# ctSkennerton/crass

Measured on AMD Instinct MI355X. Metric: reads/sec through DR search+recruit, 150bp synthetic, 1/2/4/8 MI355X, higher is better.
Workload: dtype u8; 1 GPU; 100000000 synthetic 150 bp reads, 50 seeded DRs, 1 % CRISPR reads (BASELINE.json configs[2]); pass1 + merge + pass2; total_reads=100000000, reads_per_gpu=100000000, read_len=150, n_dr=50, parallelism=read-shards x1, launcher=single context, pass1_found=563794, pass2_found=436000, patterns=13320, ac_states=0, filter_survivors=1705594, fast_filter=1, lds_automaton=2, merge_fallbacks=0

## Files before the change

### crass_amd/build.py

```python
import os
import shutil
import subprocess
import sys

HERE = os.path.dirname(os.path.abspath(__file__))
CSRC = os.path.join(HERE, "csrc")
LIB = os.path.join(HERE, "libcrass_hip.so")
SOURCES = ["kernels.hip", "pass2.hip", "sinks.hip", "dmerge.hip", "consensus.hip", "pack.hip", "fastx_scan.hip", "fastx_names.hip", "inflate.hip", "gunzip.hip", "engine.cpp", "engine_ingest.cpp", "merge.cpp", "ingest.cpp", "fastx_scan.cpp", "bgzf.cpp", "gunzip.cpp", "consensus.cpp", "group.cpp", "graph.cpp", "sdma.cpp", "pgzip.cpp"]
HEADERS = ["engine_internal.h", "engine_ctx.h", "dev_common.h", "comp_table.h", "devmem.h", "pack_text.h", "lane_find.h", "pack_launch.h", "fastx_scan.h", "fastx_launch.h", "fastx_names_launch.h", "inflate_core.h", "inflate_launch.h", "gunzip_core.h", "gunzip_launch.h", "consensus_internal.h", "merge.h", os.path.join("..", "..", "include", "crass_hip.h")]


def _hipcc():
    for cand in (os.environ.get("HIPCC"), shutil.which("hipcc"), "/opt/rocm/bin/hipcc"):
        if cand and os.path.exists(cand):
            return cand
    raise RuntimeError("hipcc not found: the MI355X engine cannot be built")


OBJ = os.path.join(CSRC, "_obj")
FLAGS = ["--offload-arch=gfx950", "-O3", "-std=c++17", "-ffp-contract=off", "-fPIC", "-Wall", "-Wno-unused-function"]
LIBS = ["-lz", "-lpthread", "-ldl"]


def _stale(target, deps):
    if not os.path.exists(target):
        return True
    t = os.path.getmtime(target)
    return any(os.path.getmtime(d) > t for d in deps)


def needs_build():
    return _stale(LIB, [os.path.join(CSRC, d) for d in SOURCES + HEADERS])


def build(force=False, verbose=False):
    if not force and not needs_build():
        return LIB
    os.makedirs(OBJ, exist_ok=True)
    hipcc = _hipcc()
    hdrs = [os.path.join(CSRC, h) for h in HEADERS]
    jobs = []
    objs = []
    for s in SOURCES:
        src, obj = os.path.join(CSRC, s), os.path.join(OBJ, s + ".o")
        objs.append(obj)
        if force or _stale(obj, [src] + hdrs):
            cmd = [hipcc] + FLAGS + ["-x", "hip", "-c", src, "-o", obj]
            if verbose:
                print(" ".join(cmd), file=sys.stderr)
            jobs.append((s, subprocess.Popen(cmd, stdout=subprocess.PIPE, stderr=subprocess.STDOUT, text=True)))
    failed = []
    for s, p in jobs:
        out, _ = p.communicate()
        if out.strip():
            print(out, file=sys.stderr, end="")
        if p.returncode:
            failed.append(s)
    if failed:
        raise RuntimeError("hipcc failed for: " + ", ".join(failed))
    tmp = LIB + ".tmp"
    cmd = [hipcc, "--offload-arch=gfx950", "-shared", "-fPIC", "-o", tmp] + objs + LIBS
    if verbose:
        print(" ".join(cmd), file=sys.stderr)
    subprocess.check_call(cmd)
    from . import vgpr_guard
    try:
        vgpr_guard.check(tmp)
    except Exception:
        os.replace(tmp, LIB + ".rejected")
        raise
    os.replace(tmp, LIB)
    return LIB


ADAPTER_DIR = os.path.join(CSRC, "adapter")
CLI = os.path.join(HERE, "crass-hip")
ADAPTER_LIB = os.path.join(HERE, "libcrass_adapter.so")


def build_adapter(force=False, verbose=False):
    build(force=force, verbose=verbose)
    srcs = [os.path.join(ADAPTER_DIR, "crass_adapter.cpp")]
    deps = srcs + [os.path.join(ADAPTER_DIR, "crass_adapter.h"), os.path.join(ADAPTER_DIR, "crass_hip_cli.cpp"), LIB]
    if not force and os.path.exists(CLI) and os.path.exists(ADAPTER_LIB) and \
            all(os.path.getmtime(d) <= min(os.path.getmtime(CLI), os.path.getmtime(ADAPTER_LIB)) for d in deps):
        return CLI
    cxx = shutil.which("g++") or "g++"
    common = [cxx, "-O2", "-std=c++17", "-Wall", "-fPIC", "-pthread"]
    rpath = ["-L" + HERE, "-lcrass_hip", "-Wl,-rpath," + HERE, "-Wl,-rpath,$ORIGIN"]
    for cmd in (common + ["-shared", "-o", ADAPTER_LIB] + srcs + rpath,
                common + ["-o", CLI, os.path.join(ADAPTER_DIR, "crass_hip_cli.cpp")] + srcs + rpath):
        if verbose:
            print(" ".join(cmd), file=sys.stderr)
        subprocess.check_call(cmd)
    return CLI


if __name__ == "__main__":
    print(build(force="--force" in sys.argv, verbose=True))
    print(build_adapter(force="--force" in sys.argv, verbose=True))
```

### crass_amd/csrc/engine.cpp

```cpp
#include "engine_ctx.h"

#include <cstdio>
#include <new>
#include <string>

void crass_hip_ctx::widen_p1() const
{
    P1Dense &D = dense;
    if (D.wide_ready) return;
    (void)wait_bulk();
    const uint64_t n = D.n;
    const uint32_t ss_cap = D.pack_ss_cap, stride = dr_stride;
    const uint8_t *hb = D.h_blob.p;
    const uint16_t *b_replen = (const uint16_t *)(hb + D.lay.replen), *b_ss = (const uint16_t *)(hb + D.lay.ss);
    const uint8_t *b_nss = hb + D.lay.nss, *b_ss8 = hb + D.lay.ss;
    D.w_replen.resize(n); D.w_nss.resize(n); D.w_ss_off.resize(n); D.w_ss.resize(n * (size_t)ss_cap);
    D.w_dr_len.resize(n); D.w_dr.resize(n * (size_t)stride);
    if (D.dr_fallback) (void)hipStreamSynchronize(copy_stream);
    else (void)wait_dx();
    const size_t per_task = 16384;
    host_parallel_for((size_t)((n + per_task - 1) / per_task), 16, [&](size_t t) {
        const uint64_t k0 = t * per_task, k1 = std::min<uint64_t>(n, k0 + per_task);
        for (uint64_t k = k0; k < k1; k++) { D.w_replen[k] = b_replen[k]; D.w_nss[k] = b_nss[k]; D.w_ss_off[k] = k * (uint64_t)ss_cap; }
        if (D.lay.ss_elem == 1) for (uint64_t i = k0 * ss_cap; i < k1 * (uint64_t)ss_cap; i++) D.w_ss[i] = b_ss8[i];
        else for (uint64_t i = k0 * ss_cap; i < k1 * (uint64_t)ss_cap; i++) D.w_ss[i] = b_ss[i];
        if (D.dr_fallback) {
            memcpy(D.w_dr.data() + k0 * (size_t)stride, D.h_dr_fb.p + k0 * (size_t)stride, (size_t)(k1 - k0) * stride);
            memcpy(D.w_dr_len.data() + k0, D.h_dr_len_fb.p + k0, (size_t)(k1 - k0) * 2);
        } else {
            for (uint64_t k = k0; k < k1; k++) {
                const uint32_t j = h_dmap.p[k];
                memcpy(D.w_dr.data() + k * (size_t)stride, h_dx_chars.p + j * (size_t)stride, stride);
                D.w_dr_len[k] = h_dx_len.p[j];
            }
        }
    });
    D.wide_ready = true;
}

static void quiesce_worker(crass_hip_ctx *c)
{
    if (c->dm.build_pending) {
        if (!c->worker.run_here_if_not_started()) c->worker.wait();
        c->dm.build_pending = false;
        (void)c->worker.take_failed();
        c->dm.br.valid = false;
        if (c->dm.br.hip) { c->last_hip = c->dm.br.hip; c->dm.br.hip = 0; }
    }
}

static bool getenv_once_copy_early()
{
    static const bool on = getenv("CRASS_COPY_EARLY") != nullptr;
    return on;
}


extern "C" {

int crass_hip_abi_version(void) { return CRASS_HIP_ABI_VERSION; }

int crassi_anchor_shape(uint32_t low_dr, uint32_t *key_bases, uint32_t *align_bases)
{
    uint32_t kb = 0, ash = 0;
    const bool ok = dm_anchor_shape(low_dr, kb, ash);
    if (key_bases) *key_bases = ok ? kb : 0u;
    if (align_bases) *align_bases = ok ? 1u << ash : 0u;
    return ok ? 1 : 0;
}

uint64_t crassi_dev_bytes_live(void) { return g_dev_bytes.load(std::memory_order_relaxed); }

void crass_default_params(crass_params *p)
{
    p->lowDRsize = 23; p->highDRsize = 47; p->lowSpacerSize = 26; p->highSpacerSize = 50;
    p->searchWindowLength = 8; p->minNumRepeats = 2; p->kmer_clust_size = 6;
}

const char *crass_hip_strerror(int s)
{
    switch (s) {
        case CRASS_OK: return "ok";
        case CRASS_ERR_INVALID_ARG: return "invalid argument";
        case CRASS_ERR_UNSUPPORTED: return "parameter outside the device path's implementation limits";
        case CRASS_ERR_NO_DEVICE: return "no usable HIP device";
        case CRASS_ERR_HIP: return "HIP runtime call failed";
        case CRASS_ERR_OOM: return "out of memory";
        case CRASS_ERR_STATE: return "call order violated";
        case CRASS_ERR_SEARCH_FATAL: return "Fatal error in search algorithm!";
        case CRASS_ERR_OVERFLOW: return "device pool overflow";
        case CRASS_ERR_IO: return "I/O error";
        case CRASS_ERR_RCCL: return "RCCL call failed (crass_hip_group_last_error())";
        default: return "unknown status";
    }
}

int crass_hip_last_hip_error(const crass_hip_ctx *ctx) { return ctx ? ctx->last_hip : 0; }
void *crass_hip_stream(const crass_hip_ctx *ctx) { return ctx ? (void *)ctx->stream : nullptr; }

int crass_hip_create(const crass_params *p, int device, crass_hip_ctx **out)
{
    if (!p || !out) return CRASS_ERR_INVALID_ARG;
    *out = nullptr;
    if (p->searchWindowLength < CRASS_HIP_MIN_WINDOW || p->searchWindowLength > CRASS_HIP_MAX_WINDOW) return CRASS_ERR_INVALID_ARG;
    if (p->lowDRsize < 8 || p->lowSpacerSize < 8) return CRASS_ERR_INVALID_ARG;
    if (p->lowDRsize >= p->highDRsize || p->lowSpacerSize >= p->highSpacerSize) return CRASS_ERR_INVALID_ARG;
    if (p->minNumRepeats < 2) return CRASS_ERR_INVALID_ARG;
    if (p->highDRsize > CRASS_HIP_MAX_DR) return CRASS_ERR_UNSUPPORTED;
    if (p->lowDRsize < 2 * p->searchWindowLength - 1) return CRASS_ERR_UNSUPPORTED;
    int ndev = 0;
    if (hipGetDeviceCount(&ndev) != hipSuccess || ndev <= 0 || device < 0 || device >= ndev) return CRASS_ERR_NO_DEVICE;
    crass_hip_ctx *c = new (std::nothrow) crass_hip_ctx();
    if (!c) return CRASS_ERR_OOM;
    c->prm = *p;
    c->device = device;
    c->dp.lowDR = p->lowDRsize; c->dp.highDR = p->highDRsize; c->dp.lowSp = p->lowSpacerSize; c->dp.highSp = p->highSpacerSize;
    c->dp.window = p->searchWindowLength; c->dp.minRepeats = p->minNumRepeats;
    uint32_t skips = p->lowDRsize - (2 * p->searchWindowLength - 1);
    if (skips < 1) skips = 1;
    c->dp.skips = skips;
    c->env.read();
    g_dev_cap.store(c->env.pool_cap_bytes, std::memory_order_relaxed);
    c->dp.debug_stop = c->env.surv_debug;
    c->dp.find_serial = c->env.lane_find_serial ? 1u : 0u;
    if (c->env.stage_timing >= 0) c->timing_level = c->env.stage_timing;
    if (c->env.no_lookback) c->lb_on = false;
    c->dr_stride = (p->highDRsize + 15u) & ~15u;
    { const hipError_t he = hipSetDevice(device);
      if (he != hipSuccess) { fprintf(stderr, "[crass_hip] hipSetDevice(%d): %s\n", device, hipGetErrorString(he)); delete c; return CRASS_ERR_NO_DEVICE; } }
    if (const char *e = getenv("CRASS_WAIT")) {
        const unsigned f = !strcmp(e, "spin") ? hipDeviceScheduleSpin : !strcmp(e, "yield") ? hipDeviceScheduleYield : !strcmp(e, "block") ? hipDeviceScheduleBlockingSync : hipDeviceScheduleAuto;
        const hipError_t fe = hipSetDeviceFlags(f);
        if (fe != hipSuccess) fprintf(stderr, "[crass_hip] hipSetDeviceFlags(%s): %s\n", e, hipGetErrorString(fe));
    }
    if (getenv("CRASS_SURV_PROF")) {
        void *pp = nullptr;
        if (hipMalloc(&pp, (192 + 2 * 16384) * 8) == hipSuccess && hipMemset(pp, 0, (192 + 2 * 16384) * 8) == hipSuccess) {
            c->dp.prof = (unsigned long long *)pp;
            const unsigned long long big = ~0ull;
            (void)hipMemcpy(c->dp.prof + 188, &big, 8, hipMemcpyHostToDevice);
        }
    }
    for (hipStream_t *sp : {&c->stream, &c->copy_stream}) {
        const hipError_t he = hipStreamCreateWithFlags(sp, hipStreamNonBlocking);
        if (he != hipSuccess) { fprintf(stderr, "[crass_hip] hipStreamCreateWithFlags on device %d: %s\n", device, hipGetErrorString(he)); delete c; return CRASS_ERR_NO_DEVICE; }
    }
    for (auto &e : c->ev) if (hipEventCreate(&e) != hipSuccess) { delete c; return CRASS_ERR_HIP; }
    if (c->h_flags.ensure(8) != hipSuccess) { delete c; return CRASS_ERR_OOM; }
    memset(c->h_flags.p, 0, 32);
    c->poll_on = getenv("CRASS_NO_POLL") == nullptr;
    if (hipEventCreateWithFlags(&c->ev_gathered, hipEventDisableTiming) != hipSuccess) { delete c; return CRASS_ERR_HIP; }
    if (hipEventCreateWithFlags(&c->ev_premerge, hipEventDisableTiming) != hipSuccess) { delete c; return CRASS_ERR_HIP; }
    c->dma = sdma_create();
    if (c->dma && !getenv("CRASS_DX_PINNED")) {
        for (auto &d : c->dma_dx) d = sdma_create();
        c->dx_via_dma = c->dma_dx[0] && c->dma_dx[1] && c->dma_dx[2];
    }
    (void)warm_dmerge_module();
    *out = c;
    return CRASS_OK;
}

int crass_hip_stream_wait_event(crass_hip_ctx *c, void *event)
{
    if (!c || !event) return CRASS_ERR_INVALID_ARG;
    (void)hipSetDevice(c->device);
    HIPCHK(c, hipStreamWaitEvent(c->stream, (hipEvent_t)event, 0));
    return CRASS_OK;
}

int crass_hip_reload_env(crass_hip_ctx *c)
{
    if (!c) return CRASS_ERR_INVALID_ARG;
    c->env.read();
    g_dev_cap.store(c->env.pool_cap_bytes, std::memory_order_relaxed);
    c->dp.debug_stop = c->env.surv_debug;
    c->dp.find_serial = c->env.lane_find_serial ? 1u : 0u;
    if (c->env.stage_timing >= 0) c->timing_level = c->env.stage_timing;
    c->lb_on = !c->env.no_lookback;
    return CRASS_OK;
}

int crass_hip_set_stage_timing(crass_hip_ctx *c, int level)
{
    if (!c || level < 0 || level > 2) return CRASS_ERR_INVALID_ARG;
    c->timing_level = level;
    return CRASS_OK;
}

int crass_hip_set_host_view(crass_hip_ctx *c, int light)
{
    if (!c || light < 0 || light > 1) return CRASS_ERR_INVALID_ARG;
    quiesce_worker(c);
    c->host_view_light = light != 0;
    if (c->host_view_light) c->dm.M.x_on = 0;
    return CRASS_OK;
}

int crass_hip_set_timing_focus(crass_hip_ctx *c, unsigned kernels)
{
    if (!c || kernels > 7u) return CRASS_ERR_INVALID_ARG;
    c->timing_focus = kernels;
    return CRASS_OK;
}

void crass_hip_destroy(crass_hip_ctx *c)
{
    if (!c) return;
    (void)hipSetDevice(c->device);
    quiesce_worker(c);
    c->worker.stop();
    if (c->stream) (void)hipStreamSynchronize(c->stream);
    if (c->copy_stream) (void)hipStreamSynchronize(c->copy_stream);
    if (c->hint_stream) (void)hipStreamSynchronize(c->hint_stream);
    (void)sdma_wait(c->dma);
    (void)c->wait_dx();
    ingest_free_all(c);
    if (getenv("CRASS_POLL_REPORT")) fprintf(stderr, "[crass_hip] stage-flag polls that ran out of their budget: %u (of %u flags)\n", c->n_poll_timeouts.load(), c->flag_seq);
    c->lb_status.release(); c->lb_ticket.release(); c->h_lb_fail.release(); c->h_flags.release();
    if (c->xchg.ev_counts) (void)hipEventDestroy(c->xchg.ev_counts);
    c->dm.release(); c->h_qblob.release(); c->xchg.send.release(); c->xchg.xinfo.release(); c->xchg.h_xinfo.release();
    c->dd_map.release(); c->dd_dx_chars.release(); c->dd_dx_len.release(); c->dd_dx_hash.release();
    c->h_dmap.release(); c->h_dx_chars.release(); c->h_dx_len.release(); c->h_dx_hash.release();
    if (c->ev_gathered) (void)hipEventDestroy(c->ev_gathered);
// ... 2274 lines not shown
```

### crass_amd/csrc/kernels.hip

```cpp
#include "dev_common.h"
#include "comp_table.h"
#include "lane_find.h"
#include <type_traits>
#include <algorithm>

namespace crass {

static __constant__ CompTable c_comp = make_comp_table();

#define FG_WAVES 4

static __device__ __forceinline__ uint32_t lds_code(const uint32_t *w, uint32_t p, uint32_t mask)
{
    uint32_t wi = p >> 4, sh = (p & 15u) * 2u;
    uint64_t v = ((uint64_t)w[wi + 1] << 32) | w[wi];
    return (uint32_t)(v >> sh) & mask;
}

__global__ __launch_bounds__(FG_WAVES * WAVE) void k_filter_general(DevReads R, DevParams P, uint64_t *hitmask,
                                                                      uint32_t lds_words_per_wave)
{
    extern __shared__ __attribute__((aligned(16))) uint32_t fg_lds[];
    const int lane = threadIdx.x & 63;
    const int wave = threadIdx.x >> 6;
    uint32_t *words = fg_lds + (size_t)wave * lds_words_per_wave;
    const uint64_t n_words = (R.n_reads + 63) / 64;
    const uint32_t w = P.window;
    const uint32_t cmask = (1u << (2 * w)) - 1u;
    for (uint64_t mw = blockIdx.x * (uint64_t)FG_WAVES + wave; mw < n_words; mw += (uint64_t)gridDim.x * FG_WAVES) {
        uint64_t bits = 0;
        for (int k = 0; k < 64; k++) {
            uint64_t r = mw * 64 + k;
            if (r >= R.n_reads) break;
            if (!P.exc_survive && rd_is_exc(R, r)) continue;
            uint32_t L = rd_len(R, r);
            int searchEnd = (int)(L - P.lowDR - P.lowSp - w - 1);
            if (searchEnd < 0) continue;
            uint32_t nw = (L + 15) >> 4;
            const uint32_t *g = R.packed + rd_word_off(R, r);
            wave_sync();
            for (uint32_t i = lane; i < nw + 1; i += 64) words[i] = (i < nw) ? g[i] : 0u;
            wave_sync();
            bool hit = false;
            for (uint32_t j = 0; j <= (uint32_t)searchEnd && !hit; j += P.skips) {
                uint32_t begin = j + P.lowDR + P.lowSp;
                uint32_t end = j + P.highDR + P.highSp + w;
                if (end >= L) end = L - 1;
                if (end < begin) end = begin;
                uint32_t sj = lds_code(words, j, cmask);
                for (uint32_t p0 = begin; p0 + w <= end; p0 += 64) {
                    uint32_t p = p0 + lane;
                    bool ok = (p + w <= end) && (lds_code(words, p, cmask) == sj);
                    if (__ballot(ok)) { hit = true; break; }
                }
            }
            if (hit) bits |= (1ull << k);
        }
        if (lane == 0) hitmask[mw] = bits;
    }
}

hipError_t launch_filter_general(const DevReads &R, const DevParams &P, uint64_t *hitmask, uint32_t max_len, hipStream_t st)
{
    uint32_t wpw = ((max_len + 15) / 16 + 2 + 3) & ~3u;
    size_t lds = (size_t)FG_WAVES * wpw * 4;
    uint64_t n_words = (R.n_reads + 63) / 64;
    uint64_t blocks = (n_words + FG_WAVES - 1) / FG_WAVES;
    if (blocks > 256 * 16) blocks = 256 * 16;
    if (blocks == 0) return hipSuccess;
    CRASS_LAUNCH(k_filter_general, dim3((unsigned)blocks), dim3(FG_WAVES * WAVE), lds, st, R, P, hitmask, wpw);
    return hipGetLastError();
}


static __device__ __forceinline__ uint32_t pk_nonzero_u16(uint32_t a)
{
    uint32_t r;
    asm("v_pk_min_u16 %0, %1, %2" : "=v"(r) : "v"(a), "v"(0x00010001u));
    return r;
}
typedef uint32_t ff_u32x4 __attribute__((ext_vector_type(4), aligned(4)));
typedef uint32_t ff_u32x2 __attribute__((ext_vector_type(2), aligned(4)));
template <int W, int N>
static __device__ __forceinline__ void ff_load_words(const DevReads &R, uint64_t r, uint32_t (&w)[N])
{
    const uint32_t *g = R.packed + r * (uint64_t)W;
#pragma unroll
    for (int i = 0; i + 4 <= W; i += 4) {
        const ff_u32x4 v = *reinterpret_cast<const ff_u32x4 *>(g + i);
        w[i] = v.x; w[i + 1] = v.y; w[i + 2] = v.z; w[i + 3] = v.w;
    }
    if ((W & 3) >= 2) {
        const ff_u32x2 v = *reinterpret_cast<const ff_u32x2 *>(g + (W & ~3));
        w[W & ~3] = v.x; w[(W & ~3) + 1] = v.y;
    }
    if (W & 1) w[W - 1] = g[W - 1];
}
template <int W>
static __device__ __forceinline__ void ff_load_row(const DevReads &R, const DevParams &P, uint64_t r, uint32_t (&w)[W], uint64_t &exc_word)
{
#pragma unroll
    for (int i = 0; i < W; i++) w[i] = 0;
    exc_word = 0;
    const uint64_t wave_word = ((uint64_t)__builtin_amdgcn_readfirstlane((uint32_t)(r >> 38)) << 32) | __builtin_amdgcn_readfirstlane((uint32_t)(r >> 6));
    if (!P.exc_survive && (wave_word << 6) < R.n_reads) {
        const uint32_t *e = R.exc_mask + 2 * wave_word;
        exc_word = (uint64_t)e[0] | ((uint64_t)e[1] << 32);
    }
    if (r < R.n_reads) ff_load_words<W>(R, r, w);
}

template <int W>
static __device__ __forceinline__ void ff_request_row(const DevReads &R, const DevParams &P, uint64_t r, uint64_t r_last, uint32_t (&w)[W], uint64_t &exc_word)
{
    uint64_t wave_word = ((uint64_t)__builtin_amdgcn_readfirstlane((uint32_t)(r >> 38)) << 32) | __builtin_amdgcn_readfirstlane((uint32_t)(r >> 6));
    if (wave_word > (r_last >> 6)) wave_word = r_last >> 6;
    const uint32_t *e = R.exc_mask + 2 * wave_word;
    const uint64_t ew = (uint64_t)e[0] | ((uint64_t)e[1] << 32);
    exc_word = P.exc_survive ? 0ull : ew;
    ff_load_words<W>(R, r < r_last ? r : r_last, w);
}

struct ff_nothing { __device__ __forceinline__ void operator()() const {} };
template <int D0, int D1, int LCT, int WX, int SW, typename F = ff_nothing>
static __device__ __forceinline__ void ff_exact_scan(const uint32_t (&w)[WX], uint32_t (&acc)[SW], F &&early = F())
{
#pragma unroll
    for (int i = 0; i < SW; i++) acc[i] = 0xFFFFFFFFu;
#pragma unroll
    for (int d = D0; d <= D1; d++) {
        if (d == D0 + 1) early();
        const int q = d >> 4;
        const int sh = (d & 15) * 2;
#pragma unroll
        for (int k = 0; k < SW; k++) {
            if (LCT > 0 && d > LCT - 9 - 16 * k) continue;
            uint32_t lo = w[k + q], hi = w[k + q + 1];
            uint32_t s = sh ? ((lo >> sh) | (hi << (32 - sh))) : lo;
            uint32_t x = s ^ w[k];
            acc[k] = pk_min_u16(acc[k], x);
        }
    }
}
template <int LCT, int SW>
static __device__ __forceinline__ uint32_t ff_exact_hint(const uint32_t (&acc)[SW], int n_seed)
{
    uint32_t t0 = 0, t1 = 0;
#pragma unroll
    for (int k = 0; k < SW; k++) {
        if (LCT > 0 && 2 * k >= n_seed) continue;
        const uint32_t f = pk_nonzero_u16(acc[k]);
        if (k < 8) t0 |= f << (2 * k); else t1 |= f << (2 * (k - 8));
    }
    uint32_t miss = (t0 | (t0 >> 15)) & 0xFFFFu;
    if (SW > 8) miss |= (t1 | (t1 >> 15)) << 16;
    return ~miss & (n_seed >= 32 ? 0xFFFFFFFFu : ((1u << n_seed) - 1u));
}

template <int W, int D0, int D1, int LCT, int RPL>
__global__ __launch_bounds__(256) void k_filter_fast_impl(DevReads R, DevParams P, uint64_t *hitmask, uint32_t *seed_hint, uint8_t *clear_found)
{
    const uint64_t r_first = blockIdx.x * (uint64_t)(256 * RPL) + threadIdx.x;
    if (clear_found && r_first == 0) clear_found[R.n_reads] = 0;
    constexpr int WX = W + (D1 >> 4) + 2;
    const uint64_t r_last = R.n_reads - 1;
    uint32_t nxt[W];
    uint64_t nxt_exc;
    if constexpr (RPL > 1) ff_request_row<W>(R, P, r_first, r_last, nxt, nxt_exc);
    else ff_load_row<W>(R, P, r_first, nxt, nxt_exc);
#pragma unroll
    for (int it = 0; it < RPL; it++) {
    const uint64_t r = r_first + (uint64_t)it * 256u;
    const bool active = r < R.n_reads;
    if constexpr (RPL == 1) { if (clear_found && active) clear_found[r] = 0; }
    uint32_t w[WX];
#pragma unroll
    for (int i = 0; i < WX; i++) w[i] = i < W ? nxt[i] : 0u;
    const bool exc = (nxt_exc >> (r & 63)) & 1u;
    if (it + 1 < RPL) {
        ff_request_row<W>(R, P, r + 256u, r_last, nxt, nxt_exc);
        __builtin_amdgcn_sched_barrier(0);
    }
    const uint32_t L = active ? rd_len(R, r) : 0u;
    constexpr int SW = ((16 * W - 58) / 8 + 2) / 2;
    uint32_t acc[SW];
    ff_exact_scan<D0, D1, LCT>(w, acc, [&]() { if constexpr (RPL > 1) { if (clear_found) clear_found[active ? r : R.n_reads] = 0; } });
    bool hit = false;
    const int searchEnd = LCT > 0 ? (LCT - D0 - 8 - 1) : (int)(L - P.lowDR - P.lowSp - 8 - 1);
    if (active && !exc && searchEnd >= 0) {
        const uint32_t hint = ff_exact_hint<LCT>(acc, searchEnd / 8 + 1);
        hit = hint != 0;
        if (hit) seed_hint[r] = hint;
    }
    uint64_t m = __ballot(hit);
    if ((threadIdx.x & 63) == 0 && active) hitmask[r >> 6] = m;
    }
}

static __device__ __forceinline__ uint32_t pk_minimum3_f16(uint32_t a, uint32_t b, uint32_t c)
{
    uint32_t r;
    asm("v_pk_minimum3_f16 %0, %1, %2, %3" : "=v"(r) : "v"(a), "v"(b), "v"(c));
    return r;
}
template <int W, int D0, int D1, int LCT, int RPL>
__global__ __launch_bounds__(256) void k_filter_fast_pairs(DevReads R, DevParams P, uint64_t *hitmask, uint32_t *seed_hint, uint8_t *clear_found)
{
    static_assert(LCT > 0 && LCT - D0 - 9 >= 0 && RPL * 256 <= 65536, "uniform length with at least one seed");
    __shared__ uint32_t q_n;
    __shared__ uint16_t q[256 * RPL];
    __shared__ uint32_t tile_mask[2 * 4 * RPL];
    const uint64_t r_block = blockIdx.x * (uint64_t)(256 * RPL);
    const uint64_t r_first = r_block + threadIdx.x;
    const uint32_t lane = threadIdx.x & 63u;
    if (clear_found && r_first == 0) clear_found[R.n_reads] = 0;
    constexpr int WX = W + (D1 >> 4) + 2;
    constexpr int SW = ((16 * W - 58) / 8 + 2) / 2;
    constexpr int n_seed = (LCT - D0 - 9) / 8 + 1;
    constexpr uint32_t M14 = 0x3FFF3FFFu;
    const uint64_t r_last = R.n_reads - 1;
    uint32_t nxt[W];
    uint64_t nxt_exc;
    ff_request_row<W>(R, P, r_first, r_last, nxt, nxt_exc);
    if (threadIdx.x < 2 * 4 * RPL) tile_mask[threadIdx.x] = 0;
    if (threadIdx.x == 0) q_n = 0;
    __syncthreads();
#pragma unroll
    for (int it = 0; it < RPL; it++) {
        const uint64_t r = r_first + (uint64_t)it * 256u;
        const bool active = r < R.n_reads;
        uint32_t w[WX];
#pragma unroll
        for (int i = 0; i < WX; i++) w[i] = i < W ? nxt[i] : 0u;
        const bool exc = (nxt_exc >> (r & 63)) & 1u;
        if (it + 1 < RPL) {
            ff_request_row<W>(R, P, r + 256u, r_last, nxt, nxt_exc);
            __builtin_amdgcn_sched_barrier(0);
        }
        uint32_t acc[SW];
#pragma unroll
        for (int i = 0; i < SW; i++) acc[i] = 0x3C003C00u;
#pragma unroll
        for (int d = D0; d <= D1; d += 2) {
            if (d == D0 + 2 && clear_found) clear_found[active ? r : R.n_reads] = 0;
#pragma unroll
            for (int k = 0; k < SW; k++) {
                if (d > LCT - 9 - 16 * k) continue;
                const int q0 = d >> 4, sh0 = (d & 15) * 2;
                const uint32_t s0 = sh0 ? __builtin_amdgcn_alignbit(w[k + q0 + 1], w[k + q0], sh0) : w[k + q0];
                const uint32_t a = (s0 ^ w[k]) & M14;
                uint32_t b = a;
                if (d + 1 <= D1 && d + 1 <= LCT - 9 - 16 * k) {
                    const int q1 = (d + 1) >> 4, sh1 = ((d + 1) & 15) * 2;
                    const uint32_t s1 = sh1 ? __builtin_amdgcn_alignbit(w[k + q1 + 1], w[k + q1], sh1) : w[k + q1];
                    b = (s1 ^ w[k]) & M14;
                }
                acc[k] = pk_minimum3_f16(acc[k], a, b);
            }
        }
        uint32_t m = 0x3C003C00u;
#pragma unroll
        for (int k = 0; 2 * k < n_seed; k += 2) m = pk_minimum3_f16(m, acc[k], 2 * (k + 1) < n_seed ? acc[k + 1] : acc[k]);
        const bool pos = active && !exc && pk_nonzero_u16(m) != 0x00010001u;
        const uint64_t pm = __ballot(pos);
        if (pm) {
            uint32_t base = 0;
            if (lane == 0) base = atomicAdd(&q_n, (uint32_t)__popcll(pm));
            base = __builtin_amdgcn_readfirstlane(base);
            const uint32_t before = __builtin_amdgcn_mbcnt_hi((uint32_t)(pm >> 32), __builtin_amdgcn_mbcnt_lo((uint32_t)pm, 0u));
            if (pos) q[base + before] = (uint16_t)(it * 256 + threadIdx.x);
        }
    }
    __syncthreads();
    const uint32_t qn = q_n;
    for (uint32_t b0 = threadIdx.x & ~63u; b0 < qn; b0 += 256u) {
        const bool have = b0 + lane < qn;
        const uint32_t loc = have ? q[b0 + lane] : 0u;
        uint32_t w[WX];
#pragma unroll
        for (int i = 0; i < WX; i++) w[i] = 0u;
        if (have) ff_load_words<W>(R, r_block + loc, w);
        uint32_t acc[SW];
        ff_exact_scan<D0, D1, LCT>(w, acc);
        const uint32_t hint = ff_exact_hint<LCT>(acc, n_seed);
        if (have && hint != 0) {
            seed_hint[r_block + loc] = hint;
            atomicOr(&tile_mask[loc >> 5], 1u << (loc & 31u));
        }
    }
    __syncthreads();
    if (threadIdx.x < 4 * RPL) {
        const uint64_t r0 = r_block + threadIdx.x * 64u;
        if (r0 < R.n_reads) hitmask[r0 >> 6] = (uint64_t)tile_mask[2 * threadIdx.x] | ((uint64_t)tile_mask[2 * threadIdx.x + 1] << 32);
    }
}

template <int W>
__global__ __launch_bounds__(256) void k_filter_fast_range(DevReads R, DevParams P, uint64_t *hitmask, uint32_t *seed_hint)
{
    const uint64_t r = blockIdx.x * (uint64_t)256 + threadIdx.x;
    constexpr int WX = 2 * W + 2;
    uint32_t row[W];
    uint64_t exc_word;
    ff_load_row<W>(R, P, r, row, exc_word);
    const bool active = r < R.n_reads;
    uint32_t w[WX];
#pragma unroll
    for (int i = 0; i < WX; i++) w[i] = i < W ? row[i] : 0u;
    const bool exc = (exc_word >> (r & 63)) & 1u;
    const uint32_t L = active ? rd_len(R, r) : 0u;
    constexpr int SW = ((16 * W - 26) / 8 + 2) / 2;
    const int D0 = (int)(P.lowDR + P.lowSp), D1 = min((int)(P.highDR + P.highSp), 16 * W + 15);
    uint32_t acc[SW];
#pragma unroll
    for (int i = 0; i < SW; i++) acc[i] = 0xFFFFFFFFu;
    const int n_seed_max = (16 * W - D0 - 9) / 8 + 1;
#pragma unroll
    for (int q = 0; q <= W; q++) {
        if (16 * q + 15 < D0 || 16 * q > D1) continue;
        const int sb_lo = max(0, D0 - 16 * q), sb_hi = min(15, D1 - 16 * q);
        for (int sb = sb_lo; sb <= sb_hi; sb++) {
            const uint32_t sh = (uint32_t)(2 * sb);
#pragma unroll
            for (int k = 0; k < SW; k++) {
                if (2 * k >= n_seed_max) continue;
                const uint32_t lo = w[k + q], hi = w[k + q + 1];
                acc[k] = pk_min_u16(acc[k], __builtin_amdgcn_alignbit(hi, lo, sh) ^ w[k]);
            }
        }
    }
    bool hit = false;
    const int searchEnd = (int)(L - P.lowDR - P.lowSp - 8 - 1);
    if (active && !exc && searchEnd >= 0) {
        const int n_seed = searchEnd / 8 + 1;
        uint32_t t0 = 0, t1 = 0;
#pragma unroll
        for (int k = 0; k < SW; k++) {
            const uint32_t f = pk_nonzero_u16(acc[k]);
            if (k < 8) t0 |= f << (2 * k); else t1 |= f << (2 * (k - 8));
        }
        uint32_t miss = (t0 | (t0 >> 15)) & 0xFFFFu;
        if (SW > 8) miss |= (t1 | (t1 >> 15)) << 16;
        const uint32_t hint = ~miss & (n_seed >= 32 ? 0xFFFFFFFFu : ((1u << n_seed) - 1u));
        hit = hint != 0;
        if (hit) seed_hint[r] = hint;
    }
    const uint64_t m = __ballot(hit);
    if ((threadIdx.x & 63) == 0 && active) hitmask[r >> 6] = m;
}

template <int W>
__global__ __launch_bounds__(256) void k_filter_fast_any(DevReads R, DevParams P, uint64_t *hitmask, uint32_t *seed_hint)
{
    const uint64_t r = blockIdx.x * (uint64_t)256 + threadIdx.x;
    constexpr int WX = 2 * W + 3;
    uint32_t row[W];
    uint64_t exc_word;
    ff_load_row<W>(R, P, r, row, exc_word);
    const bool active = r < R.n_reads;
    uint32_t w[WX];
#pragma unroll
    for (int i = 0; i < WX; i++) w[i] = i < W ? row[i] : 0u;
    const bool exc = (exc_word >> (r & 63)) & 1u;
    const uint32_t L = active ? rd_len(R, r) : 0u;
    const int D0 = (int)(P.lowDR + P.lowSp), D1 = min((int)(P.highDR + P.highSp), 16 * W + 15);
    const int wn = (int)P.window;
    const int s1 = min(1, wn - 1), s2 = min(2, wn - 1 - s1), s3 = min(4, wn - 1 - s1 - s2), s4 = wn - 1 - s1 - s2 - s3;
    uint32_t nz[W];
#pragma unroll
    for (int i = 0; i < W; i++) nz[i] = 0xFFFFFFFFu;
#pragma unroll
    for (int q = 0; q <= W; q++) {
        if (16 * q + 15 < D0 || 16 * q > D1) continue;
        const int sb_lo = max(0, D0 - 16 * q), sb_hi = min(15, D1 - 16 * q);
        for (int sb = sb_lo; sb <= sb_hi; sb++) {
            const uint32_t sh = (uint32_t)(2 * sb);
            uint32_t z[W + 1];
#pragma unroll
            for (int k = 0; k <= W; k++) {
                const uint32_t x = __builtin_amdgcn_alignbit(w[k + q + 1], w[k + q], sh) ^ w[k];
                z[k] = x | (x >> 1);
            }
#pragma unroll
            for (int k = 0; k < W; k++) z[k] |= __builtin_amdgcn_alignbit(z[k + 1], z[k], (uint32_t)(2 * s1));
            if (s2 > 0) {
                z[W] |= z[W] >> (2 * s1);
#pragma unroll
                for (int k = 0; k < W; k++) z[k] |= __builtin_amdgcn_alignbit(z[k + 1], z[k], (uint32_t)(2 * s2));
            }
            if (s3 > 0) {
                z[W] |= z[W] >> (2 * s2);
#pragma unroll
                for (int k = 0; k < W; k++) z[k] |= __builtin_amdgcn_alignbit(z[k + 1], z[k], (uint32_t)(2 * s3));
            }
            if (s4 > 0) {
                z[W] |= z[W] >> (2 * s3);
#pragma unroll
                for (int k = 0; k < W; k++) z[k] |= __builtin_amdgcn_alignbit(z[k + 1], z[k], (uint32_t)(2 * s4));
            }
#pragma unroll
            for (int k = 0; k < W; k++) nz[k] &= z[k];
        }
    }
    bool hit = false;
    const int searchEnd = (int)(L - P.lowDR - P.lowSp - P.window - 1);
    if (active && !exc && searchEnd >= 0) {
        const uint32_t skips = P.skips;
        uint32_t hint = 0, more = 0;
        uint32_t j = 0;
        for (uint32_t i = 0; j <= (uint32_t)searchEnd; i++, j += skips) {
            uint32_t word = 0;
#pragma unroll
            for (int k = 0; k < W; k++) word = (j >> 4) == (uint32_t)k ? nz[k] : word;
            const uint32_t m = ((word >> (2u * (j & 15u))) & 1u) ^ 1u;
            if (i < 32u) hint |= m << i; else more |= m;
        }
        hit = (hint | more) != 0;
        if (hit) seed_hint[r] = more ? 0xFFFFFFFFu : hint;
    }
    const uint64_t m = __ballot(hit);
    if ((threadIdx.x & 63) == 0 && active) hitmask[r >> 6] = m;
}

hipError_t launch_filter_fast(const DevReads &R, const DevParams &P, uint64_t *hitmask, uint32_t *seed_hint, hipStream_t st, uint8_t *clear_found, bool *cleared)
{
    if (cleared) *cleared = false;
    if (!R.stride_words || R.n_reads == 0) return hipErrorNotSupported;
    if (P.window != 8 || P.skips != 8) {
        if (P.window < 6 || P.window > 9 || P.skips < 1 || P.lowDR + P.lowSp < 17 || P.highDR + P.highSp < P.lowDR + P.lowSp) return hipErrorNotSupported;
        const uint64_t nb = (R.n_reads + 255) / 256;
        if (nb > 0x7FFFFFFFull) return hipErrorNotSupported;
        switch (R.stride_words) {
#define FA_CASE(WW) case WW: CRASS_LAUNCH((k_filter_fast_any<WW>), dim3((unsigned)nb), dim3(256), 0, st, R, P, hitmask, seed_hint); break;
            FA_CASE(4) FA_CASE(5) FA_CASE(6) FA_CASE(7) FA_CASE(8) FA_CASE(9) FA_CASE(10)
            FA_CASE(11) FA_CASE(12) FA_CASE(13) FA_CASE(14) FA_CASE(15) FA_CASE(16)
#undef FA_CASE
            default: return hipErrorNotSupported;
        }
        return hipGetLastError();
    }
    if (P.lowDR + P.lowSp != 49 || P.highDR + P.highSp != 97) {
        if (P.lowDR + P.lowSp < 17 || P.highDR + P.highSp < P.lowDR + P.lowSp) return hipErrorNotSupported;
        const uint64_t nb = (R.n_reads + 255) / 256;
        if (nb > 0x7FFFFFFFull) return hipErrorNotSupported;
        switch (R.stride_words) {
#define FR_CASE(WW) case WW: CRASS_LAUNCH((k_filter_fast_range<WW>), dim3((unsigned)nb), dim3(256), 0, st, R, P, hitmask, seed_hint); break;
            FR_CASE(4) FR_CASE(5) FR_CASE(6) FR_CASE(7) FR_CASE(8) FR_CASE(9) FR_CASE(10)
            FR_CASE(11) FR_CASE(12) FR_CASE(13) FR_CASE(14) FR_CASE(15) FR_CASE(16)
#undef FR_CASE
            default: return hipErrorNotSupported;
        }
        return hipGetLastError();
    }
    uint64_t blocks = (R.n_reads + 255) / 256;
    if (blocks > 0x7FFFFFFFull) return hipErrorNotSupported;
    static const int rpl_env = getenv("CRASS_FF_RPL") ? atoi(getenv("CRASS_FF_RPL")) : 0;
    const int rpl = rpl_env ? rpl_env : (R.n_reads >= (1u << 22) ? 4 : 1);
    dim3 g((unsigned)blocks), b(256), g4((unsigned)((blocks + 3) / 4));
    static const bool ff_exact = getenv("CRASS_FF_EXACT") && atoi(getenv("CRASS_FF_EXACT")) != 0;
    if (cleared && clear_found) *cleared = true;
#define FF_LEN(LL, WW) if (R.uniform_len == LL && R.stride_words == WW) { \
        if (rpl >= 4 && !ff_exact) CRASS_LAUNCH((k_filter_fast_pairs<WW, 49, 97, LL, 4>), g4, b, 0, st, R, P, hitmask, seed_hint, clear_found); \
        else if (rpl >= 4) CRASS_LAUNCH((k_filter_fast_impl<WW, 49, 97, LL, 4>), g4, b, 0, st, R, P, hitmask, seed_hint, clear_found); \
        else CRASS_LAUNCH((k_filter_fast_impl<WW, 49, 97, LL, 1>), g, b, 0, st, R, P, hitmask, seed_hint, clear_found); \
        return hipGetLastError(); }
    FF_LEN(100, 7) FF_LEN(101, 7) FF_LEN(125, 8) FF_LEN(126, 8) FF_LEN(150, 10) FF_LEN(151, 10) FF_LEN(250, 16) FF_LEN(251, 16)
#undef FF_LEN
    switch (R.stride_words) {
#define FF_CASE(WW) case WW: CRASS_LAUNCH((k_filter_fast_impl<WW, 49, 97, 0, 1>), g, b, 0, st, R, P, hitmask, seed_hint, clear_found); break;
        FF_CASE(4) FF_CASE(5) FF_CASE(6) FF_CASE(7) FF_CASE(8) FF_CASE(9) FF_CASE(10)
        FF_CASE(11) FF_CASE(12) FF_CASE(13) FF_CASE(14) FF_CASE(15) FF_CASE(16)
#undef FF_CASE
        default: if (cleared) *cleared = false; return hipErrorNotSupported;
    }
    return hipGetLastError();
}

static __device__ __forceinline__ uint64_t hint_bits_class(const uint32_t (&w)[13], uint32_t rho)
{
    uint32_t v[12];
    const uint32_t rs = 2u * rho;
#pragma unroll
    for (int i = 0; i < 12; i++) v[i] = rs ? ((w[i] >> rs) | (w[i + 1] << (32u - rs))) : w[i];
    uint32_t acc[4] = {0xFFFFFFFFu, 0xFFFFFFFFu, 0xFFFFFFFFu, 0xFFFFFFFFu};
#pragma unroll
    for (int d = 49; d <= 97; d++) {
        const int q = d >> 4, sh = (d & 15) * 2;
#pragma unroll
        for (int k = 0; k < 4; k++) {
            const uint32_t lo = v[k + q], hi = v[k + q + 1];
            const uint32_t x = (sh ? ((lo >> sh) | (hi << (32 - sh))) : lo) ^ v[k];
            acc[k] = pk_min_u16(acc[k], x);
        }
    }
    const uint32_t m0 = pk_nonzero_u16(acc[0]), m1 = pk_nonzero_u16(acc[1]), m2 = pk_nonzero_u16(acc[2]), m3 = pk_nonzero_u16(acc[3]);
    const uint32_t lo = __builtin_amdgcn_perm(m1, m0, 0x06040200u) ^ 0x01010101u;
    const uint32_t hi = __builtin_amdgcn_perm(m3, m2, 0x06040200u) ^ 0x01010101u;
    return ((uint64_t)(hi << rho) << 32) | (uint64_t)(lo << rho);
}

static __device__ __forceinline__ uint64_t hint_bits_class_range(const uint32_t (&w)[13], uint32_t rho, int D0, int D1)
{
    uint32_t v[12];
    const uint32_t rs = 2u * rho;
#pragma unroll
    for (int i = 0; i < 12; i++) v[i] = rs ? ((w[i] >> rs) | (w[i + 1] << (32u - rs))) : w[i];
    uint32_t acc[4] = {0xFFFFFFFFu, 0xFFFFFFFFu, 0xFFFFFFFFu, 0xFFFFFFFFu};
#pragma unroll
    for (int q = 0; q < 8; q++) {
        if (16 * q + 15 < D0 || 16 * q > D1) continue;
        const int sb_lo = max(0, D0 - 16 * q), sb_hi = min(15, D1 - 16 * q);
        for (int sb = sb_lo; sb <= sb_hi; sb++) {
            const uint32_t sh = (uint32_t)(2 * sb);
#pragma unroll
            for (int k = 0; k < 4; k++) acc[k] = pk_min_u16(acc[k], __builtin_amdgcn_alignbit(v[k + q + 1], v[k + q], sh) ^ v[k]);
        }
    }
    const uint32_t m0 = pk_nonzero_u16(acc[0]), m1 = pk_nonzero_u16(acc[1]), m2 = pk_nonzero_u16(acc[2]), m3 = pk_nonzero_u16(acc[3]);
    const uint32_t lo = __builtin_amdgcn_perm(m1, m0, 0x06040200u) ^ 0x01010101u;
    const uint32_t hi = __builtin_amdgcn_perm(m3, m2, 0x06040200u) ^ 0x01010101u;
    return ((uint64_t)(hi << rho) << 32) | (uint64_t)(lo << rho);
}
template <bool RANGE>
static __device__ __forceinline__ uint64_t hint_bits_any(const uint32_t (&w)[13], uint32_t rho, int D0, int D1)
{
    if (RANGE) return hint_bits_class_range(w, rho, D0, D1);
    return hint_bits_class(w, rho);
}

static __device__ __forceinline__ void hint_tile_read(const DevReads &R, const uint64_t *hint_off, const uint32_t *blk_read, uint64_t t, uint64_t n_words,
                                                      uint64_t &r, uint32_t &tile)
{
    if (R.uniform_len) {
        const uint32_t per_read = (R.uniform_len + 63u) >> 6;
        if ((n_words >> 32) == 0) {
            const uint32_t t32 = (uint32_t)t, r32 = t32 / per_read;
            r = r32;
            tile = t32 - r32 * per_read;
        } else {
            r = t / per_read;
            tile = (uint32_t)(t - r * per_read);
        }
    } else if (blk_read) {
        uint64_t lo = blk_read[t >> 8], hi = (uint64_t)blk_read[(t >> 8) + 1] + 1;
        if (hi > R.n_reads) hi = R.n_reads;
        while (hi - lo > 1) { const uint64_t mid = (lo + hi) >> 1; if (hint_off[mid] <= t) lo = mid; else hi = mid; }
        r = lo;
        tile = (uint32_t)(t - hint_off[r]);
    } else {
        uint64_t lo = 0, hi = R.n_reads;
        while (hi - lo > 1) { const uint64_t mid = (lo + hi) >> 1; if (hint_off[mid] <= t) lo = mid; else hi = mid; }
        r = lo;
        tile = (uint32_t)(t - hint_off[r]);
    }
}

template <bool RANGE>
__global__ __launch_bounds__(256) void k_hint_positions(DevReads R, const uint64_t *hint_off, const uint32_t *blk_read, uint64_t t0, uint64_t n_words, uint64_t *hint_bits,
                                                        int D0, int D1, uint64_t *hitmask, uint32_t exc_survive)
{
    const uint64_t t = t0 + blockIdx.x * (uint64_t)blockDim.x + threadIdx.x;
    if (t >= n_words) return;
    uint64_t r;
    uint32_t tile;
    hint_tile_read(R, hint_off, blk_read, t, n_words, r, tile);
    const uint32_t L = rd_len(R, r);
    const uint32_t nw = (L + 15) >> 4;
    const uint32_t *g = R.packed + rd_word_off(R, r) + tile * 4u;
    const uint32_t rem = nw - tile * 4u;
    uint32_t w[13];
    typedef uint32_t hp_u32x4 __attribute__((ext_vector_type(4), aligned(4)));
    if (__ballot(rem < 13u || r + 1 >= R.n_reads) == 0ull) {
        const hp_u32x4 a = *reinterpret_cast<const hp_u32x4 *>(g), b = *reinterpret_cast<const hp_u32x4 *>(g + 4), c4 = *reinterpret_cast<const hp_u32x4 *>(g + 8);
        w[0] = a.x; w[1] = a.y; w[2] = a.z; w[3] = a.w; w[4] = b.x; w[5] = b.y; w[6] = b.z; w[7] = b.w;
        w[8] = c4.x; w[9] = c4.y; w[10] = c4.z; w[11] = c4.w; w[12] = g[12];
    } else {
#pragma unroll
        for (int i = 0; i < 13; i++) w[i] = (uint32_t)i < rem ? g[i] : 0u;
    }
    uint64_t bits = hint_bits_any<RANGE>(w, 0u, D0, D1);
    const int last = (int)L - D0 - 9 - (int)(tile * 64u);
    bits = last < 0 ? 0ull : (last >= 63 ? bits : (bits & ((2ull << last) - 1ull)));
    hint_bits[t] = bits;
    if (hitmask && bits && (exc_survive || !rd_is_exc(R, r))) atomicOr(reinterpret_cast<unsigned long long *>(hitmask) + (r >> 6), 1ull << (r & 63u));
}

hipError_t launch_hint_positions(const DevReads &R, const DevParams &P, const uint64_t *hint_off, const uint32_t *blk_read, uint64_t n_words,
                                 uint64_t *hint_bits, hipStream_t st, uint64_t w_begin, uint64_t w_end, uint64_t *hitmask)
{
    if (P.window != 8 || P.skips != 8 || P.lowDR + P.lowSp < 17 || P.highDR + P.highSp > 127 || P.highDR + P.highSp < P.lowDR + P.lowSp) return hipErrorNotSupported;
    if (w_end > n_words) w_end = n_words;
    if ((w_begin & 255u) != 0) return hipErrorInvalidValue;
    if (w_begin >= w_end) return hipSuccess;
    const int D0 = (int)(P.lowDR + P.lowSp), D1 = (int)(P.highDR + P.highSp);
    const dim3 hg((unsigned)((w_end - w_begin + 255) / 256));
    static const int force_hp = getenv("CRASS_HINT_RANGE") ? atoi(getenv("CRASS_HINT_RANGE")) : 0;
    if (D0 == 49 && D1 == 97 && !(force_hp & 1)) CRASS_LAUNCH(k_hint_positions<false>, hg, dim3(256), 0, st, R, hint_off, blk_read, w_begin, w_end, hint_bits, D0, D1, hitmask, P.exc_survive);
    else CRASS_LAUNCH(k_hint_positions<true>, hg, dim3(256), 0, st, R, hint_off, blk_read, w_begin, w_end, hint_bits, D0, D1, hitmask, P.exc_survive);
    return hipGetLastError();
}

static __device__ __forceinline__ uint64_t hint_bits_every(const uint32_t (&w)[13], int wn, int D0, int D1)
{
    const int s1 = min(1, wn - 1), s2 = min(2, wn - 1 - s1), s3 = min(4, wn - 1 - s1 - s2), s4 = wn - 1 - s1 - s2 - s3;
    uint32_t nz[4] = {0xFFFFFFFFu, 0xFFFFFFFFu, 0xFFFFFFFFu, 0xFFFFFFFFu};
#pragma unroll
    for (int q = 0; q < 8; q++) {
        if (16 * q + 15 < D0 || 16 * q > D1) continue;
        const int sb_lo = max(0, D0 - 16 * q), sb_hi = min(15, D1 - 16 * q);
        for (int sb = sb_lo; sb <= sb_hi; sb++) {
            const uint32_t sh = (uint32_t)(2 * sb);
            uint32_t z[5];
#pragma unroll
            for (int k = 0; k < 5; k++) {
                const uint32_t x = __builtin_amdgcn_alignbit(w[k + q + 1], w[k + q], sh) ^ w[k];
// ... 2461 lines not shown
```

Baseline: 30.40 billion reads/s.

## Recheck fast-filter survivors per seed word instead of per whole row

```diff
diff --git a/crass_amd/build.py b/crass_amd/build.py
--- a/crass_amd/build.py
+++ b/crass_amd/build.py
@@ -7,7 +7,7 @@
 CSRC = os.path.join(HERE, "csrc")
 LIB = os.path.join(HERE, "libcrass_hip.so")
 SOURCES = ["kernels.hip", "pass2.hip", "sinks.hip", "dmerge.hip", "consensus.hip", "pack.hip", "fastx_scan.hip", "fastx_names.hip", "inflate.hip", "gunzip.hip", "engine.cpp", "engine_ingest.cpp", "merge.cpp", "ingest.cpp", "fastx_scan.cpp", "bgzf.cpp", "gunzip.cpp", "consensus.cpp", "group.cpp", "graph.cpp", "sdma.cpp", "pgzip.cpp"]
-HEADERS = ["engine_internal.h", "engine_ctx.h", "dev_common.h", "comp_table.h", "devmem.h", "pack_text.h", "lane_find.h", "pack_launch.h", "fastx_scan.h", "fastx_launch.h", "fastx_names_launch.h", "inflate_core.h", "inflate_launch.h", "gunzip_core.h", "gunzip_launch.h", "consensus_internal.h", "merge.h", os.path.join("..", "..", "include", "crass_hip.h")]
+HEADERS = ["engine_internal.h", "engine_ctx.h", "dev_common.h", "comp_table.h", "devmem.h", "pack_text.h", "lane_find.h", "filter_recheck.h", "pack_launch.h", "fastx_scan.h", "fastx_launch.h", "fastx_names_launch.h", "inflate_core.h", "inflate_launch.h", "gunzip_core.h", "gunzip_launch.h", "consensus_internal.h", "merge.h", os.path.join("..", "..", "include", "crass_hip.h")]
 
 
 def _hipcc():
diff --git a/crass_amd/csrc/engine.cpp b/crass_amd/csrc/engine.cpp
--- a/crass_amd/csrc/engine.cpp
+++ b/crass_amd/csrc/engine.cpp
@@ -70,6 +70,32 @@
 }
 
 uint64_t crassi_dev_bytes_live(void) { return g_dev_bytes.load(std::memory_order_relaxed); }
+
+int crassi_filter_words(crass_hip_ctx *c, uint64_t *mask_out, uint32_t *hint_out)
+{
+    if (!c || !mask_out || !hint_out) return CRASS_ERR_INVALID_ARG;
+    if (!c->have_reads) return CRASS_ERR_STATE;
+    (void)hipSetDevice(c->device);
+    (void)c->wait_bulk();
+    (void)c->wait_dx();
+    quiesce_worker(c);
+    c->have_pass1 = c->have_merge = c->have_pass2 = false;
+    c->dm.active = false;
+    c->premerge_inflight = false;
+    c->p1d.active = false;
+    c->hints_valid = false;
+    const uint64_t n = c->R.n_reads;
+    if (c->max_len > c->env.long_min || c->R.stride_words < 4 || c->R.stride_words > 16) return CRASS_ERR_UNSUPPORTED;
+    c->dp.exc_survive = (c->R.n_exc > 0 && !c->env.exc_separate) ? 1u : 0u;
+    HIPCHK(c, hipMemsetAsync(c->d_hit_info.p, 0, n * sizeof(uint32_t), c->stream));
+    const hipError_t fe = launch_filter_fast(c->R, c->dp, c->d_mask.p, c->d_hit_info.p, c->stream);
+    if (fe == hipErrorNotSupported) return CRASS_ERR_UNSUPPORTED;
+    HIPCHK(c, fe);
+    HIPCHK(c, hipMemcpyAsync(mask_out, c->d_mask.p, ((n + 63) / 64) * sizeof(uint64_t), hipMemcpyDeviceToHost, c->stream));
+    HIPCHK(c, hipMemcpyAsync(hint_out, c->d_hit_info.p, n * sizeof(uint32_t), hipMemcpyDeviceToHost, c->stream));
+    HIPCHK(c, hipStreamSynchronize(c->stream));
+    return CRASS_OK;
+}
 
 void crass_default_params(crass_params *p)
 {
diff --git a/crass_amd/csrc/filter_recheck.h b/crass_amd/csrc/filter_recheck.h
--- /dev/null
+++ b/crass_amd/csrc/filter_recheck.h
@@ -0,0 +1,68 @@
+#pragma once
+#include <stdint.h>
+
+#ifndef CRASS_HD
+#ifdef __HIPCC__
+#define CRASS_HD __host__ __device__
+#else
+#define CRASS_HD
+#endif
+#endif
+
+#ifdef __HIPCC__
+#define CRASS_FR_UNROLL _Pragma("unroll")
+#else
+#define CRASS_FR_UNROLL
+#endif
+
+namespace crass {
+
+CRASS_HD inline uint32_t fr_alignbit(uint32_t hi, uint32_t lo, uint32_t sh)
+{
+#if defined(__HIP_DEVICE_COMPILE__)
+    return __builtin_amdgcn_alignbit(hi, lo, sh);
+#else
+    return sh ? (lo >> sh) | (hi << (32u - sh)) : lo;
+#endif
+}
+
+CRASS_HD inline uint32_t fr_pk_min_u16(uint32_t a, uint32_t b)
+{
+#if defined(__HIP_DEVICE_COMPILE__)
+    uint32_t r;
+    asm("v_pk_min_u16 %0, %1, %2" : "=v"(r) : "v"(a), "v"(b));
+    return r;
+#else
+    const uint32_t al = a & 0xFFFFu, bl = b & 0xFFFFu, ah = a >> 16, bh = b >> 16;
+    return (al < bl ? al : bl) | ((ah < bh ? ah : bh) << 16);
+#endif
+}
+
+template <int D0, int D1>
+struct RecheckWords { static constexpr int first = D0 >> 4, count = (D1 >> 4) - (D0 >> 4) + 2; };
+
+template <int D1, int LCT>
+CRASS_HD inline int recheck_last_shift(int k)
+{
+    const int t = LCT - 9 - 16 * k;
+    return t < D1 ? t : D1;
+}
+
+template <int D0, int D1, int LCT>
+CRASS_HD inline uint32_t recheck_word(uint32_t wk, const uint32_t (&u)[RecheckWords<D0, D1>::count], int k)
+{
+    static_assert(D0 >= 16 && D1 >= D0 && LCT > 0, "a compile-time length and shifts of at least a word");
+    const int last = recheck_last_shift<D1, LCT>(k);
+    uint32_t acc = 0xFFFFFFFFu;
+CRASS_FR_UNROLL
+    for (int d = D0; d <= D1; d++) {
+        const bool cut = d == D0 || (LCT - 8 - d >= 0 && (LCT - 8 - d) % 16 == 0);
+        if (cut && d > last) break;
+        const int q = (d >> 4) - RecheckWords<D0, D1>::first;
+        const uint32_t x = fr_alignbit(u[q + 1], u[q], 2u * (uint32_t)(d & 15)) ^ wk;
+        acc = fr_pk_min_u16(acc, x);
+    }
+    return ((acc & 0xFFFFu) ? 0u : 1u) | ((acc >> 16) ? 0u : 2u);
+}
+
+}
diff --git a/crass_amd/csrc/kernels.hip b/crass_amd/csrc/kernels.hip
--- a/crass_amd/csrc/kernels.hip
+++ b/crass_amd/csrc/kernels.hip
@@ -1,6 +1,8 @@
 #include "dev_common.h"
 #include "comp_table.h"
 #include "lane_find.h"
+#include "filter_recheck.h"
+#include <string.h>
 #include <type_traits>
 #include <algorithm>
 
@@ -81,6 +83,8 @@
 }
 typedef uint32_t ff_u32x4 __attribute__((ext_vector_type(4), aligned(4)));
 typedef uint32_t ff_u32x2 __attribute__((ext_vector_type(2), aligned(4)));
+typedef uint32_t ff_u32x2a __attribute__((ext_vector_type(2)));
+#define FF_QCAP 128
 template <int W, int N>
 static __device__ __forceinline__ void ff_load_words(const DevReads &R, uint64_t r, uint32_t (&w)[N])
 {
@@ -204,26 +208,35 @@
     return r;
 }
 template <int W, int D0, int D1, int LCT, int RPL>
-__global__ __launch_bounds__(256) void k_filter_fast_pairs(DevReads R, DevParams P, uint64_t *hitmask, uint32_t *seed_hint, uint8_t *clear_found)
+__global__ __launch_bounds__(256) void k_filter_fast_pairs(DevReads R, DevParams P, uint64_t *hitmask, uint32_t *seed_hint, uint8_t *clear_found, uint32_t word_cap)
 {
     static_assert(LCT > 0 && LCT - D0 - 9 >= 0 && RPL * 256 <= 65536, "uniform length with at least one seed");
-    __shared__ uint32_t q_n;
+    constexpr int n_seed = (LCT - D0 - 9) / 8 + 1;
+    constexpr int NSW = (n_seed + 1) / 2;
+    constexpr int NSP = (NSW + 1) / 2;
+    static_assert(NSW <= 16 && FF_QCAP <= 256, "an entry is (queue slot, word) in 8 + 4 bits, a queue slot has one owner thread");
+    __shared__ uint32_t q_n, e_n;
     __shared__ uint16_t q[256 * RPL];
     __shared__ uint32_t tile_mask[2 * 4 * RPL];
+    __shared__ ff_u32x2a q_acc[FF_QCAP * NSP];
+    __shared__ uint32_t q_hint[FF_QCAP];
+    __shared__ uint16_t ent[FF_QCAP * NSW];
+    constexpr int RSP = (NSW + crass::RecheckWords<D0, D1>::first + crass::RecheckWords<D0, D1>::count) / 2;
+    constexpr int RS = 2 * RSP;
+    __shared__ ff_u32x2a q_row[FF_QCAP * RSP];
     const uint64_t r_block = blockIdx.x * (uint64_t)(256 * RPL);
     const uint64_t r_first = r_block + threadIdx.x;
     const uint32_t lane = threadIdx.x & 63u;
     if (clear_found && r_first == 0) clear_found[R.n_reads] = 0;
     constexpr int WX = W + (D1 >> 4) + 2;
     constexpr int SW = ((16 * W - 58) / 8 + 2) / 2;
-    constexpr int n_seed = (LCT - D0 - 9) / 8 + 1;
     constexpr uint32_t M14 = 0x3FFF3FFFu;
     const uint64_t r_last = R.n_reads - 1;
     uint32_t nxt[W];
     uint64_t nxt_exc;
     ff_request_row<W>(R, P, r_first, r_last, nxt, nxt_exc);
     if (threadIdx.x < 2 * 4 * RPL) tile_mask[threadIdx.x] = 0;
-    if (threadIdx.x == 0) q_n = 0;
+    if (threadIdx.x == 0) { q_n = 0; e_n = 0; }
     __syncthreads();
 #pragma unroll
     for (int it = 0; it < RPL; it++) {
@@ -268,12 +281,77 @@
             if (lane == 0) base = atomicAdd(&q_n, (uint32_t)__popcll(pm));
             base = __builtin_amdgcn_readfirstlane(base);
             const uint32_t before = __builtin_amdgcn_mbcnt_hi((uint32_t)(pm >> 32), __builtin_amdgcn_mbcnt_lo((uint32_t)pm, 0u));
-            if (pos) q[base + before] = (uint16_t)(it * 256 + threadIdx.x);
+            const uint32_t slot = base + before;
+            if (pos) {
+                q[slot] = (uint16_t)(it * 256 + threadIdx.x);
+                if (slot < word_cap) {
+#pragma unroll
+                    for (int k = 0; k < NSP; k++) q_acc[__umul24(slot, NSP) + k] = ff_u32x2a{acc[2 * k], 2 * k + 1 < NSW ? acc[2 * k + 1] : 0x3C003C00u};
+                }
+            }
         }
     }
     __syncthreads();
     const uint32_t qn = q_n;
-    for (uint32_t b0 = threadIdx.x & ~63u; b0 < qn; b0 += 256u) {
+    const uint32_t nw = qn < word_cap ? qn : word_cap;
+    const uint32_t wave0 = threadIdx.x & ~63u;
+    if (wave0 < nw) {
+        const bool have = threadIdx.x < nw;
+        if (have) {
+            q_hint[threadIdx.x] = 0;
+            uint32_t wr[RS > W ? RS : W];
+#pragma unroll
+            for (int i = 0; i < (RS > W ? RS : W); i++) wr[i] = 0u;
+            ff_load_words<W>(R, r_block + q[threadIdx.x], wr);
+#pragma unroll
+            for (int i = 0; i < RSP; i++) q_row[__umul24(threadIdx.x, RSP) + i] = ff_u32x2a{wr[2 * i], wr[2 * i + 1]};
+        }
+        bool wp[NSW];
+        uint64_t bm[NSW];
+        uint32_t total = 0;
+#pragma unroll
+        for (int k = 0; k < NSW; k++) {
+            const ff_u32x2a a = q_acc[__umul24(have ? threadIdx.x : 0u, NSP) + (k >> 1)];
+            wp[k] = have && pk_nonzero_u16((k & 1) ? a.y : a.x) != 0x00010001u;
+            bm[k] = __ballot(wp[k]);
+            total += (uint32_t)__popcll(bm[k]);
+        }
+        uint32_t ebase = 0;
+        if (lane == 0 && total) ebase = atomicAdd(&e_n, total);
+        ebase = __builtin_amdgcn_readfirstlane(ebase);
+#pragma unroll
+        for (int k = 0; k < NSW; k++) {
+            if (wp[k]) ent[__builtin_amdgcn_mbcnt_hi((uint32_t)(bm[k] >> 32), __builtin_amdgcn_mbcnt_lo((uint32_t)bm[k], ebase))] = (uint16_t)((threadIdx.x << 4) | (uint32_t)k);
+            ebase += (uint32_t)__popcll(bm[k]);
+        }
+    }
+    if (nw) {
+        __syncthreads();
+        const uint32_t en = e_n;
+        for (uint32_t e0 = wave0; e0 < en; e0 += 256u) {
+            typedef crass::RecheckWords<D0, D1> RW;
+            const bool have = e0 + lane < en;
+            const uint32_t e = have ? ent[e0 + lane] : 0u;
+            const uint32_t slot = e >> 4, k = e & 15u;
+            const uint32_t *row = reinterpret_cast<const uint32_t *>(q_row) + __umul24(slot, RS) + k;
+            const uint32_t wk = row[0];
+            uint32_t u[RW::count];
+#pragma unroll
+            for (int i = 0; i < RW::count; i++) u[i] = row[RW::first + i];
+            const uint32_t f = crass::recheck_word<D0, D1, LCT>(wk, u, (int)k);
+            if (have && f) atomicOr(&q_hint[slot], f << (2u * k));
+        }
+        __syncthreads();
+        if (threadIdx.x < nw) {
+            const uint32_t hint = q_hint[threadIdx.x] & (n_seed >= 32 ? 0xFFFFFFFFu : ((1u << n_seed) - 1u));
+            if (hint != 0) {
+                const uint32_t loc = q[threadIdx.x];
+                seed_hint[r_block + loc] = hint;
+                atomicOr(&tile_mask[loc >> 5], 1u << (loc & 31u));
+            }
+        }
+    }
+    for (uint32_t b0 = nw + wave0; b0 < qn; b0 += 256u) {
         const bool have = b0 + lane < qn;
         const uint32_t loc = have ? q[b0 + lane] : 0u;
         uint32_t w[WX];
@@ -458,9 +536,10 @@
     const int rpl = rpl_env ? rpl_env : (R.n_reads >= (1u << 22) ? 4 : 1);
     dim3 g((unsigned)blocks), b(256), g4((unsigned)((blocks + 3) / 4));
     static const bool ff_exact = getenv("CRASS_FF_EXACT") && atoi(getenv("CRASS_FF_EXACT")) != 0;
+    static const uint32_t ff_word_cap = (getenv("CRASS_FF_RECHECK") && !strcmp(getenv("CRASS_FF_RECHECK"), "row")) ? 0u : (uint32_t)FF_QCAP;
     if (cleared && clear_found) *cleared = true;
 #define FF_LEN(LL, WW) if (R.uniform_len == LL && R.stride_words == WW) { \
-        if (rpl >= 4 && !ff_exact) CRASS_LAUNCH((k_filter_fast_pairs<WW, 49, 97, LL, 4>), g4, b, 0, st, R, P, hitmask, seed_hint, clear_found); \
+        if (rpl >= 4 && !ff_exact) CRASS_LAUNCH((k_filter_fast_pairs<WW, 49, 97, LL, 4>), g4, b, 0, st, R, P, hitmask, seed_hint, clear_found, ff_word_cap); \
         else if (rpl >= 4) CRASS_LAUNCH((k_filter_fast_impl<WW, 49, 97, LL, 4>), g4, b, 0, st, R, P, hitmask, seed_hint, clear_found); \
         else CRASS_LAUNCH((k_filter_fast_impl<WW, 49, 97, LL, 1>), g, b, 0, st, R, P, hitmask, seed_hint, clear_found); \
         return hipGetLastError(); }
```

Result: slower. 29.97 billion reads/s (-1.4%).
